# opentrack/neuralnet-tracker-traincode

Hardware: AMD Instinct MI355X
Metric: face-crops/sec fwd+bwd @ batch 512 (higher is better)
Workload: dtype f32; 1 GPU; NetworkWithPointHead(mobilenetv1, point head on, NLL off = training-script defaults): zero_grad + fwd + multi-task loss + bwd + fused clip/Adam step; per_gpu_batch=512, global_batch=512, input=129x129x1 f32, parallelism=dp1

## Files before the change

neuralnet-tracker-traincode_amd/csrc/dwconv_tiled.hip:

```cpp
#include "ttk_common.h"
#include <type_traits>
#ifndef TTK_DW_FWD_U
#define TTK_DW_FWD_U 6
#endif
#ifndef TTK_DW_BWD_U
#define TTK_DW_BWD_U 4
#endif
#ifndef TTK_DW_FWD_U2
#define TTK_DW_FWD_U2 6
#endif

namespace ttk {

#ifndef TTK_DW_LDS_PIX
#define TTK_DW_LDS_PIX 368
#endif
constexpr int kLdsPixBudget32 = TTK_DW_LDS_PIX;
__host__ __device__ constexpr int lds_pix_budget(int SL) { return kLdsPixBudget32 * 32 / SL; }
__host__ __device__ constexpr int ilog2(int v) { return v <= 1 ? 0 : 1 + ilog2(v >> 1); }
#ifndef TTK_DW_WGS_PER_CU
#define TTK_DW_WGS_PER_CU 3
#endif
constexpr int kMaxDwBlocks = 256 * TTK_DW_WGS_PER_CU;
constexpr int kFwdUSkip = 4, kFwdUPlain = TTK_DW_FWD_U, kFwdUPlain2 = TTK_DW_FWD_U2;

struct DwTiling {
  int SL;
  int R, nbands, nslabs, grid, rows;
  int NI;
  int stage_rows;
  int NCT, TW;
  int carry;
};
#ifndef TTK_DW_CARRY
#define TTK_DW_CARRY 1
#endif
#ifndef TTK_DW_CARRY_BWD
#define TTK_DW_CARRY_BWD 1
#endif
constexpr int kCarryRegs = 5;

constexpr int kColTileMinW = 48;
constexpr int kColTile = 17;

__host__ __device__ inline int dw_band_rows(int Hgrid, int Wstage, int stride, bool backward, int SL = 32) {
  const int stage_rows = lds_pix_budget(SL) / (Wstage + 2);
  int R;
  if (!backward) R = (stage_rows - 3) / stride + 1;
  else R = (stride == 1) ? stage_rows - 2 : 2 * (stage_rows - 2);
  if (R < 1) R = 1;
  if (R > Hgrid) R = Hgrid;
  return R;
}

inline DwTiling dw_tiling_sl(int B, int H, int W, int C, int stride, bool backward, int SL) {
  const int Ho = (H - 1) / stride + 1, Wo = (W - 1) / stride + 1;
  DwTiling t;
  t.SL = SL;
  t.NCT = 1;
  t.TW = Wo;
  t.carry = backward ? (TTK_DW_CARRY_BWD && stride == 1 && (Wo + 2) <= 80)
                     : (TTK_DW_CARRY && (3 - stride) * (W + 2) * (SL / 4) <= kCarryRegs * kBlock);
  if (!t.carry && stride == 1 && W >= kColTileMinW) {
    t.NCT = (W + kColTile - 1) / kColTile;
    t.TW = (W + t.NCT - 1) / t.NCT;
  }
  const int Wtile = t.NCT > 1 ? t.TW : (backward ? Wo : W);
  t.R = backward ? dw_band_rows(H, Wtile, stride, true, SL) : dw_band_rows(Ho, Wtile, stride, false, SL);
  t.nbands = ((backward ? H : Ho) + t.R - 1) / t.R;
  t.nslabs = C / SL;
  t.stage_rows = backward ? (stride == 1 ? t.R + 2 : t.R / 2 + 2) : (t.R - 1) * stride + 3;
  t.NI = 1;
  if (t.nbands == 1) t.carry = 0;
  if (t.nbands == 1 && t.NCT == 1) {
    const int per_image = t.stage_rows * ((backward ? Wo : W) + 2);
    t.NI = lds_pix_budget(SL) / per_image;
    if (t.NI > B) t.NI = B;
    if (t.NI < 1) t.NI = 1;
  }
  int64_t tiles_per_slab = (int64_t)((B + t.NI - 1) / t.NI) * t.nbands * t.NCT;
  int64_t rows = kMaxDwBlocks / t.nslabs;
  if (rows < 1) rows = 1;
  if (rows > tiles_per_slab) rows = tiles_per_slab;
  t.rows = (int)rows;
  t.grid = t.rows * t.nslabs;
  return t;
}

inline DwTiling dw_tiling(int B, int H, int W, int C, int stride, bool backward) {
  return dw_tiling_sl(B, H, W, C, stride, backward, kCB);
}

struct TileDiv {
  float inv;
  unsigned d;
  __device__ __forceinline__ explicit TileDiv(unsigned d_) : inv(1.0f / (float)d_), d(d_) {}
  __device__ __forceinline__ unsigned div(unsigned n) const { return (unsigned)(((float)n + 0.5f) * inv); }
};

struct SlabWeights {
  float v[36];
  __device__ __forceinline__ void load(const float* w, int c) {
    const float4* p = reinterpret_cast<const float4*>(w + 9 * c);
#pragma unroll
    for (int i = 0; i < 9; ++i) {
      const float4 q = p[i];
      v[4 * i] = q.x; v[4 * i + 1] = q.y; v[4 * i + 2] = q.z; v[4 * i + 3] = q.w;
    }
  }
  __device__ __forceinline__ float4 tap(int t) const { return make_float4(v[t], v[9 + t], v[18 + t], v[27 + t]); }
};

template <int SL>
__device__ __forceinline__ float4 slab_wave_fold(float4 v) {
#pragma unroll
  for (int off = SL / 4; off < kWave; off <<= 1) {
    v.x += __shfl_xor(v.x, off); v.y += __shfl_xor(v.y, off);
    v.z += __shfl_xor(v.z, off); v.w += __shfl_xor(v.w, off);
  }
  return v;
}

struct D4 {
  double x, y, z, w;
  __device__ __forceinline__ void add(float4 v) { x += v.x; y += v.y; z += v.z; w += v.w; }
  __device__ __forceinline__ void addmul(float4 a, float4 b) {
    x += (double)a.x * b.x; y += (double)a.y * b.y; z += (double)a.z * b.z; w += (double)a.w * b.w;
  }
};
__device__ __forceinline__ double shfl_xor_d(double v, int off) {
  int lo = __double2loint(v), hi = __double2hiint(v);
  lo = __shfl_xor(lo, off);
  hi = __shfl_xor(hi, off);
  return __hiloint2double(hi, lo);
}
template <int SL>
__device__ __forceinline__ D4 slab_wave_fold_d(D4 v) {
#pragma unroll
  for (int off = SL / 4; off < kWave; off <<= 1) {
    v.x += shfl_xor_d(v.x, off); v.y += shfl_xor_d(v.y, off);
    v.z += shfl_xor_d(v.z, off); v.w += shfl_xor_d(v.w, off);
  }
  return v;
}

template <int SL>
__device__ __forceinline__ void slab_partials(D4 s1, D4 s2, int q, int C, int c_slab, float* part_row, float* red_f) {
  double* red = reinterpret_cast<double*>(red_f);
  s1 = slab_wave_fold_d<SL>(s1);
  s2 = slab_wave_fold_d<SL>(s2);
  const int lane = threadIdx.x & 63, wv = threadIdx.x >> 6;
  __syncthreads();
  if (lane < SL / 4) {
    double* d = red + (wv * 2 + 0) * SL + 4 * q;
    d[0] = s1.x; d[1] = s1.y; d[2] = s1.z; d[3] = s1.w;
    d = red + (wv * 2 + 1) * SL + 4 * q;
    d[0] = s2.x; d[1] = s2.y; d[2] = s2.z; d[3] = s2.w;
  }
  __syncthreads();
  if (threadIdx.x < 2 * SL) {
    const int which = threadIdx.x / SL, c = threadIdx.x % SL;
    double a = 0.0;
    for (int w = 0; w < kBlock / kWave; ++w) a += red[(w * 2 + which) * SL + c];
    part_row[(size_t)which * C + c_slab + c] = (float)a;
  }
}

enum { kSkipNone = 0, kSkipStored = 1, kSkipRaw = 2 };
__device__ __forceinline__ const float* only_ptr(const float* p) { return p; }

template <int S, int SKIP, int SL, bool CARRY, typename... BnSkip>
__global__ void __launch_bounds__(kBlock) __attribute__((amdgpu_waves_per_eu(TTK_DW_WGS_PER_CU, TTK_DW_WGS_PER_CU)))
dw_fwd_tiled_k(const float* __restrict__ yprev, const float* __restrict__ bn_prev,
                                                          const float* __restrict__ skip_prev, float* __restrict__ a_out,
                                                          const float* __restrict__ w, float* __restrict__ y,
                                                          float* __restrict__ part, const float* __restrict__ pivot, int B, int H, int W, int C,
                                                          int Ho, int Wo, int R, int nbands, int nslabs, int NI_, int NCT_, int TW, BnSkip... bn_skip) {
  static_assert(sizeof...(BnSkip) == (SKIP == kSkipRaw ? 1 : 0), "bn_skip: the raw residual form's one extra argument");
  extern __shared__ __attribute__((aligned(16))) float lds[];
  constexpr int kSlab = SL, kSlabQuads = SL / 4, kPixSlots = kBlock / kSlabQuads, kQs = ilog2(kSlabQuads), kPs = ilog2(SL);
  const int tid = threadIdx.x, q = tid & (kSlabQuads - 1), slot = tid >> kQs;
  const int slab = blockIdx.x % nslabs, c0 = slab * kSlab + 4 * q;
  static_assert(SL == kCB, "a slab is one channel block of the activation layout");
  constexpr int cshift = 5;
  SlabWeights wr;
  wr.load(w, c0);
  const BnApply4 bn = BnApply4::load(bn_prev, C, c0);
  BnApply4 bns = bn;
  if constexpr (SKIP == kSkipRaw) bns = BnApply4::load(only_ptr(bn_skip...), C, c0);
  const float4 pv = pivot ? ld4(pivot + c0) : f4(0.f);
  D4 s1{0.0, 0.0, 0.0, 0.0}, s2{0.0, 0.0, 0.0, 0.0};
  const int NI = CARRY ? 1 : NI_, NCT = CARRY ? 1 : NCT_;
  constexpr bool carry = CARRY;
  const unsigned tiles = (unsigned)((B + NI - 1) / NI) * nbands * NCT;
  const unsigned wgs = gridDim.x / nslabs, wg = blockIdx.x / nslabs;
  const unsigned t_begin = carry ? (unsigned)((uint64_t)tiles * wg / wgs) : wg, t_end = carry ? (unsigned)((uint64_t)tiles * (wg + 1) / wgs) : tiles;
  const unsigned t_step = carry ? 1u : wgs;
  int prev_img = -1, prev_band = -2, prev_nrows = 0;
  constexpr int OV = 3 - S;
  for (unsigned t = t_begin; t < t_end; t += t_step) {
    const unsigned tb = t / (unsigned)NCT, ti = tb / (unsigned)nbands;
    const int ct = (int)(t - tb * NCT), band = (int)(tb - ti * nbands), n0 = (int)ti * NI;
    const int nimg = min(NI, B - n0);
    const int cx0 = ct * TW, tw = NCT > 1 ? min(TW, Wo - cx0) : Wo;
    const int Wp = NCT > 1 ? tw + 2 : W + 2;
    const int o0 = band * R, o1 = min(o0 + R, Ho);
    const int i0 = o0 * S - 1;
    const int nrows = (o1 - 1 - o0) * S + 3;
    const unsigned PI = (unsigned)(nrows * Wp);
    const TileDiv dPI(PI), dWp((unsigned)Wp), dtw((unsigned)tw);
    const size_t tin = ((size_t)slab * B * H * W + (size_t)n0 * H * W) * kCB, tout = ((size_t)slab * B * Ho * Wo + (size_t)n0 * Ho * Wo) * kCB;
    const float* ytile = yprev + tin;
    const float* sktile = SKIP ? skip_prev + tin : nullptr;
    float* aotile = a_out ? a_out + tin : nullptr;
    float* youttile = y + tout;
    const int ov = (carry && (int)ti == prev_img && band == prev_band + 1) ? OV : 0;
    const int own_hi = (carry && t + 1 < t_end && band + 1 < nbands) ? i0 + nrows : o1;
    float4 cr[kCarryRegs];
    const int ncopy = ov * Wp * kSlabQuads;
    if (ov) {
      const float* src = lds + (size_t)(prev_nrows - OV) * Wp * kSlab;
#pragma unroll
      for (int u = 0; u < kCarryRegs; ++u)
        if (tid + u * kBlock < ncopy) cr[u] = ld4(src + (size_t)(tid + u * kBlock) * 4);
    }
    prev_img = (int)ti; prev_band = band; prev_nrows = nrows;
    __syncthreads();
    if (ov) {
#pragma unroll
      for (int u = 0; u < kCarryRegs; ++u)
        if (tid + u * kBlock < ncopy) st4(lds + (size_t)(tid + u * kBlock) * 4, cr[u]);
    }
    const int nstage = nimg * ((int)PI - ov * Wp) * kSlabQuads;
    const unsigned ovpix = (unsigned)(ov * Wp);
    constexpr int kFwdU = SKIP ? (SKIP == kSkipRaw && S == 1 && CARRY ? kFwdUSkip - 1 : kFwdUSkip) : (S == 2 ? kFwdUPlain2 : (CARRY ? kFwdUPlain - 1 : kFwdUPlain));
    for (int e = tid; e < nstage; e += kFwdU * kBlock) {
      float4 yv[kFwdU], sk[SKIP ? kFwdU : 1];
      unsigned off[kFwdU];
      bool in[kFwdU];
      int pxs[kFwdU], rows[kFwdU];
#pragma unroll
      for (int u = 0; u < kFwdU; ++u) {
        const int ee = e + u * kBlock;
        const unsigned pxa = ((unsigned)ee >> kQs) + ovpix;
        const unsigned img = NI > 1 ? dPI.div(pxa) : 0u, px = NI > 1 ? pxa - __umul24(img, PI) : pxa;
        const unsigned prow = dWp.div(px);
        const int col = (int)(px - __umul24(prow, (unsigned)Wp)) - 1 + cx0, row = i0 + (int)prow;
        pxs[u] = (int)pxa;
        rows[u] = (row >= o0 && row < own_hi && col >= cx0 && col < cx0 + tw) ? 1 : 0;
        in[u] = ee < nstage && row >= 0 && row < H && col >= 0 && col < W;
        off[u] = in[u] ? ((__umul24(__umul24(img, (unsigned)H) + (unsigned)row, (unsigned)W) + (unsigned)col) << cshift) + 4 * q : 0u;
        yv[u] = in[u] ? ld4nt(ytile + off[u]) : f4(0.f);
        if constexpr (SKIP) sk[u] = in[u] ? ld4nt(sktile + off[u]) : f4(0.f);
      }
#pragma unroll
      for (int u = 0; u < kFwdU; ++u) {
        const int ee = e + u * kBlock;
        if (ee >= nstage) break;
        float4 a = f4(0.f);
        if (in[u]) {
          if constexpr (SKIP == kSkipRaw) a = bn.act(yv[u], bns.act(sk[u]));
          else if constexpr (SKIP == kSkipStored) a = bn.act(yv[u], sk[u]);
          else a = bn.act(yv[u]);
          if (S == 1 && a_out && rows[u]) st4(aotile + off[u], a);
        }
        st4(lds + (size_t)pxs[u] * kSlab + 4 * q, a);
      }
    }
    __syncthreads();
    const unsigned npix1 = (unsigned)((o1 - o0) * tw);
    const int npix = nimg * (int)npix1;
    const TileDiv dnp(npix1);
    for (int p = slot; p < npix; p += kPixSlots) {
      const unsigned img = NI > 1 ? dnp.div((unsigned)p) : 0u, pp = NI > 1 ? (unsigned)p - __umul24(img, npix1) : (unsigned)p;
      const unsigned prow = dtw.div(pp);
      const int ho = o0 + (int)prow, wl = (int)(pp - __umul24(prow, (unsigned)tw)), wo = cx0 + wl;
      const float* base = lds + ((__umul24(img, PI) + __umul24(prow * S, (unsigned)Wp) + (unsigned)(wl * S)) << kPs) + 4 * q;
      float4 acc = f4(0.f);
#pragma unroll
      for (int kh = 0; kh < 3; ++kh)
#pragma unroll
        for (int kw = 0; kw < 3; ++kw) acc = fma4(ld4(base + ((size_t)kh * Wp + kw) * kSlab), wr.tap(kh * 3 + kw), acc);
      st4(youttile + ((__umul24(__umul24(img, (unsigned)Ho) + (unsigned)ho, (unsigned)Wo) + (unsigned)wo) << cshift) + 4 * q, acc);
      acc = sub4(acc, pv);
      s1.add(acc);
      s2.addmul(acc, acc);
    }
  }
  if (part) {
    const int stage = NI * ((R - 1) * S + 3) * (NCT > 1 ? TW + 2 : W + 2) * kSlab;
    slab_partials<SL>(s1, s2, q, C, slab * kSlab, part + (size_t)(blockIdx.x / nslabs) * 2 * C, lds + stage);
  }
}

#ifndef TTK_DW_BWD_LEAN_PIX
#define TTK_DW_BWD_LEAN_PIX 4
#endif
#ifndef TTK_DW_BWD_LEAN_PIX2
#define TTK_DW_BWD_LEAN_PIX2 4
#endif
template <int S, int SL, bool LEAN, bool CARRY, typename... BnSkip>
__global__ void __launch_bounds__(kBlock) __attribute__((amdgpu_waves_per_eu(TTK_DW_WGS_PER_CU, TTK_DW_WGS_PER_CU)))
dw_bwd_tiled_k(const float* __restrict__ g_dw, const float* __restrict__ y_dw,
                                                          const float* __restrict__ bn_dw, const float* __restrict__ w,
                                                          const float* __restrict__ skip_grad,
                                                          const float* __restrict__ yprev, float* __restrict__ bn_prev,
                                                          const float* __restrict__ skip_prev, const float* __restrict__ a_in,
                                                          float* __restrict__ g_prev, float* __restrict__ part,
                                                          float* __restrict__ dwgrad, float* __restrict__ dw_partial, int B, int H, int W, int C, int Ho, int Wo,
                                                          int R, int nbands, int nslabs, int stage_floats, int NI_, int NCT_, int TW, int ring, BnSkip... bn_skip) {
  constexpr bool RAWSKIP = sizeof...(BnSkip) == 1;
  static_assert(sizeof...(BnSkip) <= 1 && !(RAWSKIP && LEAN), "bn_skip: the raw residual form's one extra argument");
  extern __shared__ __attribute__((aligned(16))) float lds[];
  const int NI = CARRY ? 1 : NI_, NCT = CARRY ? 1 : NCT_;
  constexpr int kSlab = SL, kSlabQuads = SL / 4, kPixSlots = kBlock / kSlabQuads, kQs = ilog2(kSlabQuads), kPs = ilog2(SL);
  const int tid = threadIdx.x, q = tid & (kSlabQuads - 1), slot = tid >> kQs;
  const int slab = blockIdx.x % nslabs, c0 = slab * kSlab + 4 * q;
  float* wt = lds + stage_floats + 4 * 9 * kSlab;
  if (slot == 0) {
#pragma unroll
    for (int t = 0; t < 9; ++t)
      st4(wt + t * kSlab + 4 * q, make_float4(w[(size_t)(c0 + 0) * 9 + t], w[(size_t)(c0 + 1) * 9 + t], w[(size_t)(c0 + 2) * 9 + t], w[(size_t)(c0 + 3) * 9 + t]));
  }
  static_assert(SL == kCB, "a slab is one channel block of the activation layout");
  constexpr int cshift = 5;
  const BnApply4 bnp = BnApply4::load(bn_prev, C, c0);
  BnApply4 bns = bnp;
  if constexpr (RAWSKIP) bns = BnApply4::load(only_ptr(bn_skip...), C, c0);
  const BnGrad4 bg = BnGrad4::load(bn_dw, C, c0);
  D4 s1{0.0, 0.0, 0.0, 0.0}, s2{0.0, 0.0, 0.0, 0.0};
  float gmx = 0.f;
  float4 wacc[9];
#pragma unroll
  for (int t = 0; t < 9; ++t) wacc[t] = f4(0.f);
  const unsigned tiles = (unsigned)((B + NI - 1) / NI) * nbands * NCT;
  const unsigned wgs = gridDim.x / nslabs, wg = blockIdx.x / nslabs;
  const unsigned t_begin = CARRY ? (unsigned)((uint64_t)tiles * wg / wgs) : wg, t_end = CARRY ? (unsigned)((uint64_t)tiles * (wg + 1) / wgs) : tiles;
  const unsigned t_step = CARRY ? 1u : wgs;
  int prev_img = -1, prev_band = -2, prev_hi = -1;
  for (unsigned t = t_begin; t < t_end; t += t_step) {
    const unsigned tb = t / (unsigned)NCT, ti = tb / (unsigned)nbands;
    const int ct = (int)(t - tb * NCT), band = (int)(tb - ti * nbands), n0 = (int)ti * NI;
    const int nimg = min(NI, B - n0);
    const int cx0 = ct * TW, tw = NCT > 1 ? min(TW, W - cx0) : W;
    const int Wp = NCT > 1 ? tw + 2 : Wo + 2;
    const int r0 = band * R, r1 = min(r0 + R, H);
    const int ho_lo = max(0, (r0 - 1 + S - 1) / S * (r0 > 0 ? 1 : 0));
    const int ho_hi = min(Ho - 1, r1 / S);
    const int nrows = ho_hi - ho_lo + 1;
    const unsigned PI = (unsigned)(nrows * Wp);
    const TileDiv dPI(PI), dWp((unsigned)Wp), dtw((unsigned)tw);
    const size_t tdy = ((size_t)slab * B * Ho * Wo + (size_t)n0 * Ho * Wo) * kCB, tin = ((size_t)slab * B * H * W + (size_t)n0 * H * W) * kCB;
    const float* gtile = g_dw + tdy;
    const float* ydtile = y_dw + tdy;
    const float* yptile = yprev + tin;
    const float* aitile = a_in ? a_in + tin : nullptr;
    const float* sktile = skip_prev ? skip_prev + tin : nullptr;
    const float* sgtile = skip_grad ? skip_grad + tin : nullptr;
    float* gptile = g_prev + tin;
    const int ov = (CARRY && (int)ti == prev_img && band == prev_band + 1 && prev_hi >= ho_lo) ? prev_hi - ho_lo + 1 : 0;
    const int rbase = CARRY ? ho_lo % ring : 0;
    prev_img = (int)ti; prev_band = band; prev_hi = ho_hi;
    __syncthreads();
    const unsigned ovpix = (unsigned)(ov * Wp);
    const int nstage = nimg * ((int)PI - (int)ovpix) * kSlabQuads;
    constexpr int kBwdU = (RAWSKIP && S == 1 && !CARRY) ? TTK_DW_BWD_U - 2 : TTK_DW_BWD_U;
    for (int e = tid; e < nstage; e += kBwdU * kBlock) {
      float4 gv[kBwdU], yv[kBwdU];
      bool in[kBwdU];
      unsigned pxs[kBwdU];
#pragma unroll
      for (int u = 0; u < kBwdU; ++u) {
        const int ee = e + u * kBlock;
        const unsigned pxa = ((unsigned)ee >> kQs) + ovpix;
        const unsigned img = NI > 1 ? dPI.div(pxa) : 0u, px = NI > 1 ? pxa - __umul24(img, PI) : pxa;
        const unsigned prow = dWp.div(px);
        const int col = (int)(px - __umul24(prow, (unsigned)Wp)) - 1 + cx0, row = ho_lo + (int)prow;
        if constexpr (CARRY) {
          unsigned rr = (unsigned)rbase + prow;
          rr -= rr >= (unsigned)ring ? (unsigned)ring : 0u;
          pxs[u] = __umul24(rr, (unsigned)Wp) + (px - __umul24(prow, (unsigned)Wp));
        } else {
          pxs[u] = pxa;
        }
        in[u] = ee < nstage && col >= 0 && col < Wo;
        const unsigned off = in[u] ? ((__umul24(__umul24(img, (unsigned)Ho) + (unsigned)row, (unsigned)Wo) + (unsigned)col) << cshift) + 4 * q : 0u;
        gv[u] = in[u] ? ld4nt(gtile + off) : f4(0.f);
        yv[u] = in[u] ? ld4nt(ydtile + off) : f4(0.f);
      }
#pragma unroll
      for (int u = 0; u < kBwdU; ++u) {
        const int ee = e + u * kBlock;
        if (ee >= nstage) break;
        st4(lds + (size_t)pxs[u] * kSlab + 4 * q, in[u] ? bg.dy(gv[u], yv[u]) : f4(0.f));
      }
    }
    __syncthreads();
    const unsigned npix1 = (unsigned)((r1 - r0) * tw);
    const int npix = nimg * (int)npix1;
    const TileDiv dnp(npix1);
    constexpr int NP = LEAN ? (S == 2 ? TTK_DW_BWD_LEAN_PIX2 : TTK_DW_BWD_LEAN_PIX) : 2;
    for (int p = slot; p < npix; p += NP * kPixSlots) {
      bool has[NP];
      unsigned imgs[NP], offs[NP];
      int his[NP], wis[NP];
      float4 yps[NP], raws[NP], sgs[NP];
#pragma unroll
      for (int j = 0; j < NP; ++j) {
        const int pj = p + j * kPixSlots;
        has[j] = pj < npix;
        const unsigned pq = has[j] ? (unsigned)pj : (unsigned)p;
        imgs[j] = NI > 1 ? dnp.div(pq) : 0u;
        const unsigned pp = NI > 1 ? pq - __umul24(imgs[j], npix1) : pq;
        const unsigned pr = dtw.div(pp);
        his[j] = r0 + (int)pr;
        wis[j] = cx0 + (int)(pp - __umul24(pr, (unsigned)tw));
        offs[j] = ((__umul24(__umul24(imgs[j], (unsigned)H) + (unsigned)his[j], (unsigned)W) + (unsigned)wis[j]) << cshift) + 4 * q;
      }
#pragma unroll
      for (int j = 0; j < NP; ++j) yps[j] = ld4nt(yptile + offs[j]);
#pragma unroll
      for (int j = 0; j < NP; ++j) {
        raws[j] = f4(0.f);
        sgs[j] = f4(0.f);
        if (!LEAN) {
          if (a_in) raws[j] = ld4nt(aitile + offs[j]);
          else if (skip_prev) raws[j] = ld4nt(sktile + offs[j]);
          if (skip_grad) sgs[j] = ld4nt(sgtile + offs[j]);
        }
      }
#pragma unroll
      for (int j = 0; j < NP; ++j) {
        if (j > 0 && !has[j]) break;
        const int hi = his[j], wi = wis[j];
        const float* dyimg = lds + (__umul24(imgs[j], PI) << kPs);
        const float4 yp = yps[j], raw = raws[j], sg = sgs[j];
        float4 a;
        if constexpr (RAWSKIP) a = bnp.act(yp, bns.act(raw));
        else if (!LEAN && a_in) a = raw;
        else a = (!LEAN && skip_prev) ? bnp.act(yp, raw) : bnp.act(yp);
        float4 G = f4(0.f);
#pragma unroll
        for (int kh = 0; kh < 3; ++kh) {
          const int th = hi + 1 - kh;
          if (th < 0 || (S == 2 && (th & 1))) continue;
          const int ho = th / S;
          if (ho > Ho - 1) continue;
#pragma unroll
          for (int kw = 0; kw < 3; ++kw) {
            const int tw = wi + 1 - kw;
            if (S == 2 && (tw & 1)) continue;
            const int wo = (S == 1) ? tw : (tw >> 1);
            int lr = ho - ho_lo;
            if constexpr (CARRY) { lr += rbase; lr -= lr >= ring ? ring : 0; }
            const float4 dy = ld4(dyimg + ((__mul24(lr, Wp) + wo - cx0 + 1) << kPs) + 4 * q);
            G = fma4(dy, ld4(wt + (kh * 3 + kw) * kSlab + 4 * q), G);
            wacc[kh * 3 + kw] = fma4(dy, a, wacc[kh * 3 + kw]);
          }
        }
        if (!LEAN && skip_grad) G = add4(G, sg);
        const float4 gp = mask4(G, a);
        st4(gptile + offs[j], gp);
        gmx = fmaxf(fmaxf(gmx, fmaxf(fabsf(gp.x), fabsf(gp.y))), fmaxf(fabsf(gp.z), fabsf(gp.w)));
        s1.add(gp);
        s2.addmul(gp, sub4(yp, bnp.mean));
      }
    }
  }
  float* red = lds + stage_floats;
#pragma unroll
  for (int off = 32; off >= 1; off >>= 1) gmx = fmaxf(gmx, __shfl_xor(gmx, off));
  if ((tid & 63) == 0) {
    unsigned* slot = reinterpret_cast<unsigned*>(bn_prev + (size_t)TTK_BN_AUX * C + TTK_AUX_GMAX);
    if (__float_as_uint(gmx) > __hip_atomic_load(slot, __ATOMIC_RELAXED, __HIP_MEMORY_SCOPE_AGENT)) atomicMax(slot, __float_as_uint(gmx));
  }
  if (part) slab_partials<SL>(s1, s2, q, C, slab * kSlab, part + (size_t)(blockIdx.x / nslabs) * 2 * C, red);
  if (dwgrad) {
    __syncthreads();
    const int lane = tid & 63, wv = tid >> 6;
#pragma unroll
    for (int t = 0; t < 9; ++t) {
      const float4 v = slab_wave_fold<SL>(wacc[t]);
      if (lane < kSlabQuads) st4(red + ((size_t)wv * 9 + t) * kSlab + 4 * q, v);
    }
    __syncthreads();
    for (int i = tid; i < 9 * kSlab; i += kBlock) {
      const int t = i / kSlab, c = i % kSlab;
      float a = 0.f;
      for (int wq = 0; wq < kBlock / kWave; ++wq) a += red[((size_t)wq * 9 + t) * kSlab + c];
      if (dw_partial) dw_partial[((size_t)(blockIdx.x / nslabs) * C + slab * kSlab + c) * 9 + t] = a;
      else atomicAdd(dwgrad + (size_t)(slab * kSlab + c) * 9 + t, a);
    }
  }
}

__global__ void zero_fill_k(float* p, int64_t n) {
  const int64_t i = (int64_t)blockIdx.x * blockDim.x + threadIdx.x;
  if (i < n) p[i] = 0.f;
}

template <typename F>
static void with_flag(bool b, F&& f) {
  if (b) f(std::true_type{});
  else f(std::false_type{});
}

static bool dw_shape_ok2(int B, int H, int W, int C, int stride) {
  return B > 0 && H > 0 && W > 0 && W <= 256 && C >= 32 && C <= 1024 && (C & (C - 1)) == 0 && (stride == 1 || stride == 2);
}

constexpr size_t kMaxDynLds = 64 * 1024;
static size_t dw_fwd_lds_bytes(const DwTiling& t, int W) {
  const size_t stage = (size_t)t.NI * t.stage_rows * ((t.NCT > 1 ? t.TW : W) + 2) * t.SL;
  return (stage + 16 * t.SL) * sizeof(float);
}

}

using namespace ttk;

extern "C" {

int ttk_partial_rows_dwconv(int B, int H, int W, int C, int stride, int backward) {
  if (!dw_shape_ok2(B, H, W, C, stride)) return -1;
  const DwTiling t = dw_tiling(B, H, W, C, stride, backward != 0);
  if (!backward && dw_fwd_lds_bytes(t, W) > kMaxDynLds) return -1;
  return t.rows;
}

static int dw_fwd_launch(const char* name, bool raw, const float* yprev, const float* bn_prev, const float* skip_prev, const float* skip_bn, float* a_out,
                         const float* w, float* y, float* part, const float* pivot, int B, int H, int W, int C, int stride, int act_bf16, ttk_stream_t stream) {
  TTK_REQUIRE(yprev && bn_prev && w && y && (!raw || (skip_prev && skip_bn)), "%s: null pointer", name);
  TTK_REQUIRE(dw_shape_ok2(B, H, W, C, stride), "%s: unsupported shape B=%d H=%d W=%d C=%d stride=%d (C: power of two in 32..1024, W <= 256)", name, B, H, W, C, stride);
  TTK_REQUIRE(!(a_out && stride != 1), "%s: a_out requires stride 1", name);
  TTK_REQUIRE((act_bf16 & 3) == 0, "%s: bf16 activation storage under the fp32 kernels was retired (round 6): use the bf16-compute path (ttk_bc_*)", name);
  const int Ho = (H - 1) / stride + 1, Wo = (W - 1) / stride + 1;
  const DwTiling t = dw_tiling(B, H, W, C, stride, false);
  TTK_REQUIRE((int64_t)((B + t.NI - 1) / t.NI) * t.nbands * t.NCT < ((int64_t)1 << 31), "%s: too many tiles for 32-bit indexing", name);
  const size_t sm = dw_fwd_lds_bytes(t, W);
  TTK_REQUIRE(sm <= kMaxDynLds, "%s: unsupported shape W=%d stride=%d: the stage of %zu bytes exceeds the 64 KiB of LDS of a workgroup (stride-2 forward: W <= 163)",
              name, W, stride, sm);
  with_flag(stride == 2, [&](auto s2) {
    with_flag(t.carry != 0, [&](auto carry) {
      constexpr int S = decltype(s2)::value ? 2 : 1;
      constexpr bool CARRY = decltype(carry)::value;
      if (raw) {
        hipLaunchKernelGGL((dw_fwd_tiled_k<S, kSkipRaw, kCB, CARRY, const float*>), dim3(t.grid), dim3(kBlock), sm, (hipStream_t)stream, yprev, bn_prev, skip_prev,
                           a_out, w, y, part, pivot, B, H, W, C, Ho, Wo, t.R, t.nbands, t.nslabs, t.NI, t.NCT, t.TW, skip_bn);
      } else {
        with_flag(skip_prev != nullptr, [&](auto skip) {
          hipLaunchKernelGGL((dw_fwd_tiled_k<S, decltype(skip)::value ? kSkipStored : kSkipNone, kCB, CARRY>), dim3(t.grid), dim3(kBlock), sm, (hipStream_t)stream, yprev, bn_prev, skip_prev,
                             a_out, w, y, part, pivot, B, H, W, C, Ho, Wo, t.R, t.nbands, t.nslabs, t.NI, t.NCT, t.TW);
        });
      }
    });
  });
  TTK_LAUNCH_CHECK(name);
}

int ttk_dwconv3x3_fwd(const float* yprev, const float* bn_prev, const float* skip_prev, float* a_out, const float* w, float* y,
                      float* part, const float* pivot, int B, int H, int W, int C, int stride, int act_bf16, ttk_stream_t stream) {
  return dw_fwd_launch("dwconv3x3_fwd", false, yprev, bn_prev, skip_prev, nullptr, a_out, w, y, part, pivot, B, H, W, C, stride, act_bf16, stream);
}

int ttk_dwconv3x3_fwd_rawskip(const float* yprev, const float* bn_prev, const float* skip_raw, const float* skip_bn, float* a_out, const float* w, float* y,
                              float* part, const float* pivot, int B, int H, int W, int C, int stride, ttk_stream_t stream) {
  return dw_fwd_launch("dwconv3x3_fwd_rawskip", true, yprev, bn_prev, skip_raw, skip_bn, a_out, w, y, part, pivot, B, H, W, C, stride, 0, stream);
}

static int dw_bwd_launch(const char* name, bool raw, const float* g_dw, const float* y_dw, const float* bn_dw, const float* w, const float* skip_grad,
                         const float* yprev, float* bn_prev, const float* skip_prev, const float* skip_bn, const float* a_in, float* g_prev, float* part, float* dw,
                         int dw_accumulate, float* dw_partial, int B, int H, int W, int C, int stride, int act_bf16, ttk_stream_t stream) {
  TTK_REQUIRE(g_dw && y_dw && bn_dw && w && yprev && bn_prev && g_prev && (!raw || (skip_prev && skip_bn)), "%s: null pointer", name);
  TTK_REQUIRE(dw_shape_ok2(B, H, W, C, stride), "%s: unsupported shape", name);
  TTK_REQUIRE(!(skip_grad && stride != 1), "%s: residual gradient requires stride 1", name);
  TTK_REQUIRE((act_bf16 & 3) == 0, "%s: bf16 activation storage under the fp32 kernels was retired (round 6): use the bf16-compute path (ttk_bc_*)", name);
  const int Ho = (H - 1) / stride + 1, Wo = (W - 1) / stride + 1;
  const DwTiling t = dw_tiling(B, H, W, C, stride, true);
  TTK_REQUIRE((int64_t)((B + t.NI - 1) / t.NI) * t.nbands * t.NCT < ((int64_t)1 << 31), "%s: too many tiles for 32-bit indexing", name);
  const size_t stage = (size_t)t.NI * t.stage_rows * ((t.NCT > 1 ? t.TW : Wo) + 2) * t.SL;
  const size_t sm = (stage + 4 * 9 * t.SL + 9 * t.SL) * sizeof(float);
  hipStream_t st = (hipStream_t)stream;
  if (!dw) dw_partial = nullptr;
  TTK_REQUIRE(dw_accumulate != 2 || dw_partial, "%s: dw_accumulate = 2 (rows folded by the caller) needs dw and dw_partial", name);
  if (dw && !dw_accumulate && !dw_partial) hipLaunchKernelGGL(zero_fill_k, dim3((9 * C + 255) / 256), dim3(256), 0, st, dw, (int64_t)9 * C);
  with_flag(stride == 2, [&](auto s2) {
    with_flag(t.carry != 0, [&](auto carry) {
      constexpr int S = decltype(s2)::value ? 2 : 1;
      constexpr bool CARRY = decltype(carry)::value;
      if (raw) {
        hipLaunchKernelGGL((dw_bwd_tiled_k<S, kCB, false, CARRY, const float*>), dim3(t.grid), dim3(kBlock), sm, st, g_dw, y_dw, bn_dw, w, skip_grad, yprev, bn_prev,
                           skip_prev, a_in, g_prev, part, dw, dw_partial, B, H, W, C, Ho, Wo, t.R, t.nbands, t.nslabs, (int)stage, t.NI, t.NCT, t.TW, t.stage_rows,
                           skip_bn);
      } else {
        with_flag(!a_in && !skip_prev && !skip_grad, [&](auto lean) {
          hipLaunchKernelGGL((dw_bwd_tiled_k<S, kCB, decltype(lean)::value, CARRY>), dim3(t.grid), dim3(kBlock), sm, st, g_dw, y_dw, bn_dw, w, skip_grad, yprev,
                             bn_prev, skip_prev, a_in, g_prev, part, dw, dw_partial, B, H, W, C, Ho, Wo, t.R, t.nbands, t.nslabs, (int)stage, t.NI, t.NCT, t.TW,
                             t.stage_rows);
        });
      }
    });
  });
  if (dw_partial && dw_accumulate != 2) launch_fold_partials(dw_partial, t.rows, (int64_t)9 * C, dw, dw_accumulate, st);
  TTK_LAUNCH_CHECK(name);
}

int ttk_dwconv3x3_bwd_data(const float* g_dw, const float* y_dw, const float* bn_dw, const float* w, const float* skip_grad,
                           const float* yprev, float* bn_prev, const float* skip_prev, const float* a_in, float* g_prev,
                           float* part, float* dw, int dw_accumulate, float* dw_partial, int B, int H, int W, int C, int stride,
                           int act_bf16, ttk_stream_t stream) {
  return dw_bwd_launch("dwconv3x3_bwd_data", false, g_dw, y_dw, bn_dw, w, skip_grad, yprev, bn_prev, skip_prev, nullptr, a_in, g_prev, part, dw, dw_accumulate,
                       dw_partial, B, H, W, C, stride, act_bf16, stream);
}

int ttk_dwconv3x3_bwd_data_rawskip(const float* g_dw, const float* y_dw, const float* bn_dw, const float* w, const float* skip_grad,
                                   const float* yprev, float* bn_prev, const float* skip_raw, const float* skip_bn, float* g_prev,
                                   float* part, float* dw, int dw_accumulate, float* dw_partial, int B, int H, int W, int C, int stride,
                                   ttk_stream_t stream) {
  return dw_bwd_launch("dwconv3x3_bwd_data_rawskip", true, g_dw, y_dw, bn_dw, w, skip_grad, yprev, bn_prev, skip_raw, skip_bn, nullptr, g_prev, part, dw,
                       dw_accumulate, dw_partial, B, H, W, C, stride, 0, stream);
}

}
```

Before: 73950 crops/s.

## Add quad-based stride-2 depthwise backward path and rebalance image batching

For the stride-2 depthwise conv backward pass, adds a QUAD variant. Each thread handles a 2x2 input quad, reusing four staged output-gradient values for all nine taps instead of gathering per input pixel. BN-grad constants are moved into LDS so they do not occupy registers across the loop. The tiling now lowers images-per-tile when that reduces the per-workgroup tile count under the block cap, to balance load. The new path adds code complexity and changes register pressure and scheduling (sched barriers).

```diff
diff --git a/neuralnet-tracker-traincode_amd/csrc/dwconv_tiled.hip b/neuralnet-tracker-traincode_amd/csrc/dwconv_tiled.hip
--- a/neuralnet-tracker-traincode_amd/csrc/dwconv_tiled.hip
+++ b/neuralnet-tracker-traincode_amd/csrc/dwconv_tiled.hip
@@ -77,6 +77,11 @@
     t.NI = lds_pix_budget(SL) / per_image;
     if (t.NI > B) t.NI = B;
     if (t.NI < 1) t.NI = 1;
+    const int cap = kMaxDwBlocks / t.nslabs > 1 ? kMaxDwBlocks / t.nslabs : 1;
+    const auto span = [&](int ni) { return ((B + ni - 1) / ni + cap - 1) / cap * ni; };
+    if (backward && stride == 2 && (B + t.NI - 1) / t.NI > cap)
+      for (int ni = t.NI - 1; ni >= 1; --ni)
+        if (span(ni) < span(t.NI)) t.NI = ni;
   }
   int64_t tiles_per_slab = (int64_t)((B + t.NI - 1) / t.NI) * t.nbands * t.NCT;
   int64_t rows = kMaxDwBlocks / t.nslabs;
@@ -299,7 +304,7 @@
 #ifndef TTK_DW_BWD_LEAN_PIX2
 #define TTK_DW_BWD_LEAN_PIX2 4
 #endif
-template <int S, int SL, bool LEAN, bool CARRY, typename... BnSkip>
+template <int S, int SL, bool LEAN, bool CARRY, bool QUAD, typename... BnSkip>
 __global__ void __launch_bounds__(kBlock) __attribute__((amdgpu_waves_per_eu(TTK_DW_WGS_PER_CU, TTK_DW_WGS_PER_CU)))
 dw_bwd_tiled_k(const float* __restrict__ g_dw, const float* __restrict__ y_dw,
                                                           const float* __restrict__ bn_dw, const float* __restrict__ w,
@@ -328,6 +333,16 @@
   BnApply4 bns = bnp;
   if constexpr (RAWSKIP) bns = BnApply4::load(only_ptr(bn_skip...), C, c0);
   const BnGrad4 bg = BnGrad4::load(bn_dw, C, c0);
+  constexpr bool BG_LDS = QUAD && !LEAN;
+  float* bgl = wt + 9 * kSlab;
+  if constexpr (BG_LDS) {
+    if (slot == 0) {
+      st4(bgl + 0 * kSlab + 4 * q, bg.ga);
+      st4(bgl + 1 * kSlab + 4 * q, bg.gb);
+      st4(bgl + 2 * kSlab + 4 * q, bg.gmean);
+      st4(bgl + 3 * kSlab + 4 * q, bg.mean);
+    }
+  }
   D4 s1{0.0, 0.0, 0.0, 0.0}, s2{0.0, 0.0, 0.0, 0.0};
   float gmx = 0.f;
   float4 wacc[9];
@@ -388,14 +403,99 @@
         gv[u] = in[u] ? ld4nt(gtile + off) : f4(0.f);
         yv[u] = in[u] ? ld4nt(ydtile + off) : f4(0.f);
       }
+      BnGrad4 bgs = bg;
+      if constexpr (BG_LDS) bgs = BnGrad4{ld4(bgl + 0 * kSlab + 4 * q), ld4(bgl + 1 * kSlab + 4 * q), ld4(bgl + 2 * kSlab + 4 * q), ld4(bgl + 3 * kSlab + 4 * q)};
 #pragma unroll
       for (int u = 0; u < kBwdU; ++u) {
         const int ee = e + u * kBlock;
         if (ee >= nstage) break;
-        st4(lds + (size_t)pxs[u] * kSlab + 4 * q, in[u] ? bg.dy(gv[u], yv[u]) : f4(0.f));
+        st4(lds + (size_t)pxs[u] * kSlab + 4 * q, in[u] ? bgs.dy(gv[u], yv[u]) : f4(0.f));
       }
     }
     __syncthreads();
+    if constexpr (QUAD) {
+      static_assert(S == 2 && !CARRY, "quads: the stride-2 tilings (full-width bands that start at an even row, no ring)");
+      const unsigned nq1 = (unsigned)(((r1 - r0 + 1) >> 1) * Wo);
+      const int nq = nimg * (int)nq1;
+      const TileDiv dnq(nq1), dqw((unsigned)Wo);
+      for (int p = slot; p < nq; p += kPixSlots) {
+        const unsigned img = NI > 1 ? dnq.div((unsigned)p) : 0u, pp = NI > 1 ? (unsigned)p - __umul24(img, nq1) : (unsigned)p;
+        const unsigned qi = dqw.div(pp), qj = pp - __umul24(qi, (unsigned)Wo);
+        const int hi = r0 + 2 * (int)qi, wi = 2 * (int)qj;
+        const bool hr = hi + 1 < r1, hc = wi + 1 < W;
+        const bool dr = (r0 >> 1) + (int)qi + 1 <= ho_hi;
+        const unsigned off0 = ((__umul24(__umul24(img, (unsigned)H) + (unsigned)hi, (unsigned)W) + (unsigned)wi) << cshift) + 4 * q;
+        const unsigned dcol = hc ? 1u << cshift : 0u, drow = hr ? (unsigned)W << cshift : 0u;
+        const unsigned offs[4] = {off0, off0 + dcol, off0 + drow, off0 + drow + dcol};
+        float4 yps[4], raws[4];
+        const auto load_row = [&](int j0) {
+#pragma unroll
+          for (int j = j0; j < j0 + 2; ++j) yps[j] = ld4nt(yptile + offs[j]);
+#pragma unroll
+          for (int j = j0; j < j0 + 2; ++j) {
+            raws[j] = f4(0.f);
+            if (!LEAN) {
+              if (a_in) raws[j] = ld4nt(aitile + offs[j]);
+              else if (skip_prev) raws[j] = ld4nt(sktile + offs[j]);
+            }
+          }
+        };
+        load_row(2);
+        if (LEAN) load_row(0);
+        const float* dyq = lds + ((__umul24(img, PI) + __umul24(qi, (unsigned)Wp) + qj + 1u) << kPs) + 4 * q;
+        const float4 d00 = ld4(dyq), d01 = ld4(dyq + kSlab);
+        const float4 d10 = dr ? ld4(dyq + (Wp << kPs)) : f4(0.f), d11 = dr ? ld4(dyq + (Wp << kPs) + kSlab) : f4(0.f);
+        const auto wtap = [&](int t) { return ld4(wt + t * kSlab + 4 * q); };
+        const auto block_input = [&](int j, bool has) {
+          float4 a;
+          if constexpr (RAWSKIP) a = bnp.act(yps[j], bns.act(raws[j]));
+          else if (!LEAN && a_in) a = raws[j];
+          else a = (!LEAN && skip_prev) ? bnp.act(yps[j], raws[j]) : bnp.act(yps[j]);
+          return has ? a : f4(0.f);
+        };
+        const auto finish = [&](int j, bool has, float4 G, float4 a) {
+          const float4 gp = mask4(G, a);
+          if (has) st4(gptile + offs[j], gp);
+          gmx = fmaxf(fmaxf(gmx, fmaxf(fabsf(gp.x), fabsf(gp.y))), fmaxf(fabsf(gp.z), fabsf(gp.w)));
+          s1.add(gp);
+          s2.addmul(gp, sub4(yps[j], bnp.mean));
+        };
+        {
+          const float4 a = block_input(3, hr && hc);
+          const float4 G = fma4(d00, wtap(8), fma4(d01, wtap(6), dr ? fma4(d10, wtap(2), fma4(d11, wtap(0), f4(0.f))) : f4(0.f)));
+          wacc[0] = fma4(d11, a, wacc[0]);
+          wacc[2] = fma4(d10, a, wacc[2]);
+          wacc[6] = fma4(d01, a, wacc[6]);
+          wacc[8] = fma4(d00, a, wacc[8]);
+          finish(3, hr && hc, G, a);
+        }
+        __builtin_amdgcn_sched_barrier(0);
+        {
+          const float4 a = block_input(2, hr);
+          const float4 G = fma4(d00, wtap(7), dr ? fma4(d10, wtap(1), f4(0.f)) : f4(0.f));
+          wacc[1] = fma4(d10, a, wacc[1]);
+          wacc[7] = fma4(d00, a, wacc[7]);
+          finish(2, hr, G, a);
+        }
+        __builtin_amdgcn_sched_barrier(0);
+        if (!LEAN) load_row(0);
+        {
+          const float4 a = block_input(1, hc);
+          const float4 G = fma4(d00, wtap(5), fma4(d01, wtap(3), f4(0.f)));
+          wacc[3] = fma4(d01, a, wacc[3]);
+          wacc[5] = fma4(d00, a, wacc[5]);
+          finish(1, hc, G, a);
+        }
+        __builtin_amdgcn_sched_barrier(0);
+        {
+          const float4 a = block_input(0, true);
+          const float4 G = fma4(d00, wtap(4), f4(0.f));
+          wacc[4] = fma4(d00, a, wacc[4]);
+          finish(0, true, G, a);
+        }
+      }
+      continue;
+    }
     const unsigned npix1 = (unsigned)((r1 - r0) * tw);
     const int npix = nimg * (int)npix1;
     const TileDiv dnp(npix1);
@@ -579,22 +679,24 @@
   const DwTiling t = dw_tiling(B, H, W, C, stride, true);
   TTK_REQUIRE((int64_t)((B + t.NI - 1) / t.NI) * t.nbands * t.NCT < ((int64_t)1 << 31), "%s: too many tiles for 32-bit indexing", name);
   const size_t stage = (size_t)t.NI * t.stage_rows * ((t.NCT > 1 ? t.TW : Wo) + 2) * t.SL;
-  const size_t sm = (stage + 4 * 9 * t.SL + 9 * t.SL) * sizeof(float);
+  const bool quads = stride == 2 && !t.carry && (t.nbands == 1 || t.R % 2 == 0);
+  const size_t sm = (stage + 4 * 9 * t.SL + 9 * t.SL + (quads ? 4 * t.SL : 0)) * sizeof(float);
   hipStream_t st = (hipStream_t)stream;
   if (!dw) dw_partial = nullptr;
   TTK_REQUIRE(dw_accumulate != 2 || dw_partial, "%s: dw_accumulate = 2 (rows folded by the caller) needs dw and dw_partial", name);
   if (dw && !dw_accumulate && !dw_partial) hipLaunchKernelGGL(zero_fill_k, dim3((9 * C + 255) / 256), dim3(256), 0, st, dw, (int64_t)9 * C);
   with_flag(stride == 2, [&](auto s2) {
-    with_flag(t.carry != 0, [&](auto carry) {
+    with_flag(stride == 2 ? quads : t.carry != 0, [&](auto form) {
       constexpr int S = decltype(s2)::value ? 2 : 1;
-      constexpr bool CARRY = decltype(carry)::value;
+      constexpr bool CARRY = S == 1 && decltype(form)::value;
+      constexpr bool QUAD = S == 2 && decltype(form)::value;
       if (raw) {
-        hipLaunchKernelGGL((dw_bwd_tiled_k<S, kCB, false, CARRY, const float*>), dim3(t.grid), dim3(kBlock), sm, st, g_dw, y_dw, bn_dw, w, skip_grad, yprev, bn_prev,
+        hipLaunchKernelGGL((dw_bwd_tiled_k<S, kCB, false, CARRY, QUAD, const float*>), dim3(t.grid), dim3(kBlock), sm, st, g_dw, y_dw, bn_dw, w, skip_grad, yprev, bn_prev,
                            skip_prev, a_in, g_prev, part, dw, dw_partial, B, H, W, C, Ho, Wo, t.R, t.nbands, t.nslabs, (int)stage, t.NI, t.NCT, t.TW, t.stage_rows,
                            skip_bn);
       } else {
         with_flag(!a_in && !skip_prev && !skip_grad, [&](auto lean) {
-          hipLaunchKernelGGL((dw_bwd_tiled_k<S, kCB, decltype(lean)::value, CARRY>), dim3(t.grid), dim3(kBlock), sm, st, g_dw, y_dw, bn_dw, w, skip_grad, yprev,
+          hipLaunchKernelGGL((dw_bwd_tiled_k<S, kCB, decltype(lean)::value, CARRY, QUAD>), dim3(t.grid), dim3(kBlock), sm, st, g_dw, y_dw, bn_dw, w, skip_grad, yprev,
                              bn_prev, skip_prev, a_in, g_prev, part, dw, dw_partial, B, H, W, C, Ho, Wo, t.R, t.nbands, t.nslabs, (int)stage, t.NI, t.NCT, t.TW,
                              t.stage_rows);
         });
```

Result: no change. 74160 crops/s (median of 4 runs) (+0.3%).
